# PRONTOLab/GB-25

Measured on AMD Instinct MI355X. Metric: model time-steps/sec, higher is better.
Workload: dtype f32; 1 GPU; baroclinic_instability_model 1440x720x48 LatitudeLongitudeGrid, halo 8, SplitExplicit(30), WENO5, TEOS10, dt=120s; cells_per_gpu=49766400, local_columns=1440, local_rows=720, parallelism=single GPU, rccl_ranks=0

## Files before the change

### gb-25_amd/binding.py

```python
import ctypes as C
import os

import numpy as np

_HERE = os.path.dirname(os.path.abspath(__file__))
LIB_PATH = os.environ.get("GB25_LIB") or os.path.join(_HERE, "libgb25hip.so")
LIB_PATHS = {"Float32": LIB_PATH, "Float64": os.path.join(_HERE, "libgb25hip_f64.so")}
DTYPES = {"Float32": np.float32, "Float64": np.float64}

FIELD_IDS = {
    "u": 0, "v": 1, "w": 2, "T": 3, "S": 4, "pHY": 5,
    "Gn.u": 6, "Gn.v": 7, "Gn.T": 8, "Gn.S": 9,
    "Gm.u": 10, "Gm.v": 11, "Gm.T": 12, "Gm.S": 13,
    "eta": 14, "U": 15, "V": 16,
    "eta_bar": 17, "U_bar": 18, "V_bar": 19,
    "Gn.U": 20, "Gn.V": 21,
    "e": 22, "Gn.e": 23, "Gm.e": 24, "kappa_u": 25, "kappa_c": 26, "kappa_e": 27, "Le": 28, "Jb": 29,
    "previous_u": 30, "previous_v": 31,
}
METRIC2_IDS = ["dxfc", "dxcc", "dxcf", "dxff", "dyfc", "dycc", "dycf", "dyff", "azcc", "azfc", "azcf", "azff", "fff", "phicc"]
METRIC_IDS = {"phif": 0, "phic": 1, "dxc": 2, "dxf": 3, "azc": 4, "azf": 5, "fcor": 6,
              "zf": 7, "zc": 8, "dzc": 9, "dzf": 10, "dy": 11}
ATMOSPHERE_IDS = {"u": 0, "v": 1, "T": 2, "q": 3, "p": 4, "shortwave": 5, "longwave": 6}
KERNEL_IDS = {"fill_halos": 0, "compute_w": 1, "compute_p": 2, "gu": 3, "gv": 4, "tracers": 5,
              "ab2_velocities": 6, "ab2_tracers": 7, "barotropic": 8, "corrector": 9, "implicit": 10, "closure": 11,
              "fluxes": 12, "diagnostics": 13}

ABI_SYMBOLS = [
    "gb25_default_config", "gb25_create", "gb25_destroy", "gb25_last_error_string", "gb25_version",
    "gb25_real_bytes", "gb25_config_bytes", "gb25_catke_parameters_bytes",
    "gb25_set_stream", "gb25_use_own_stream", "gb25_synchronize", "gb25_field_dims", "gb25_set_field", "gb25_get_field",
    "gb25_field_device_ptr", "gb25_get_metric", "gb25_get_metric2", "gb25_get_substepping", "gb25_set_vertical_diffusivity",
    "gb25_get_vertical_diffusivity", "gb25_set_closure_catke", "gb25_set_prescribed_atmosphere",
    "gb25_compute_atmosphere_ocean_fluxes", "gb25_get_top_flux", "gb25_default_catke_parameters",
    "gb25_set_catke_parameters", "gb25_get_catke_parameters", "gb25_set_bottom_drag", "gb25_get_bottom_drag", "gb25_set_tracer_advection_order",
    "gb25_get_tracer_advection_order",
    "gb25_set_baroclinic_instability",
    "gb25_get_clock", "gb25_set_dt", "gb25_initialize", "gb25_mask_immersed_fields",
    "gb25_fill_halo_regions", "gb25_compute_auxiliaries", "gb25_fill_diffusivity_halos",
    "gb25_compute_momentum_tendencies", "gb25_compute_tracer_tendencies", "gb25_compute_boundary_tendencies",
    "gb25_compute_tendencies", "gb25_ab2_step", "gb25_correct_velocities_and_cache_previous_tendencies",
    "gb25_update_state", "gb25_first_time_step", "gb25_time_step", "gb25_loop",
    "gb25_set_option", "gb25_get_option", "gb25_set_bottom_height", "gb25_set_curvilinear_grid", "gb25_set_vertical_faces", "gb25_get_bottom_info", "gb25_set_top_flux",
    "gb25_comm_unique_id", "gb25_comm_init_rccl", "gb25_comm_init_local", "gb25_comm_init_callback", "gb25_comm_finalize",
    "gb25_comm_info", "gb25_debug_exchange_plan",
    "gb25_lookahead_state", "gb25_debug_sequence", "gb25_save_state",
    "gb25_profile_enable", "gb25_profile_reset", "gb25_profile_get",
    "gb25_field_stats_bytes", "gb25_field_diff_bytes", "gb25_state_monitor_bytes", "gb25_get_field_stats", "gb25_compare_field",
    "gb25_get_state_monitor", "gb25_field_device_ptr_readonly",
    "gb25_integrate_field", "gb25_get_budget", "gb25_moments_bytes", "gb25_budget_bytes",
    "gb25_derived_dims", "gb25_compute_derived", "gb25_get_derived", "gb25_get_derived_stats", "gb25_get_field_levels",
    "gb25_transport_bytes", "gb25_get_transport",
    "gb25_class_sum_bytes", "gb25_get_class_sums",
    "gb25_spectral_coefficient_bytes", "gb25_get_spectrum_table", "gb25_get_zonal_spectrum", "gb25_get_derived_zonal_spectrum",
    "gb25_compute_on_surfaces", "gb25_get_on_surfaces",
    "gb25_stability_dims", "gb25_compute_stability", "gb25_get_stability", "gb25_get_stability_stats",
    "gb25_block_info_bytes", "gb25_block_dims", "gb25_derived_block_dims", "gb25_get_block_sums", "gb25_compute_block_sums",
    "gb25_get_derived_block_sums",
    "gb25_averages_info_bytes", "gb25_averages_begin", "gb25_averages_accumulate", "gb25_averages_get_info", "gb25_average_dims",
    "gb25_get_average", "gb25_average_device_ptr", "gb25_averages_end",
    "gb25_particles_info_bytes", "gb25_particles_begin", "gb25_particles_set", "gb25_particles_get", "gb25_particles_advance",
    "gb25_particles_sample", "gb25_particles_get_info", "gb25_particles_end",
]
DERIVED_IDS = {"vorticity": 0, "kinetic_energy": 1, "density_anomaly": 2, "potential_density": 3, "mixed_layer_depth": 4}
SUM_SHAPES = {"rows": 0, "levels": 1, "total": 2}
TRANSPORT_FACES = {"across_y": 0, "across_x": 1}
TRANSPORT_SHAPES = {"lines": 0, "profile": 1, "streamfunction": 2}
CLASS_WHAT = {"faces_y": 0, "cells": 1}
CLASS_VARIABLES = {"T": 0, "S": 1, "potential_density": 2}
# ... 255 lines not shown
    lib.gb25_set_dt.argtypes = [P, C.c_double]
    lib.gb25_ab2_step.argtypes = [P, C.c_double, C.c_int]
    lib.gb25_correct_velocities_and_cache_previous_tendencies.argtypes = [P, C.c_double]
    lib.gb25_loop.argtypes = [P, C.c_int32]
    lib.gb25_save_state.argtypes = [P, C.c_char_p, C.c_char_p]
    lib.gb25_set_top_flux.argtypes = [P, C.c_int, P]
    lib.gb25_set_bottom_height.argtypes = [P, P]
    lib.gb25_set_curvilinear_grid.argtypes = [P, P, C.c_int32, C.c_int32]
    lib.gb25_set_vertical_faces.argtypes = [P, C.POINTER(C.c_double), C.c_int32]
    lib.gb25_get_bottom_info.argtypes = [P, C.c_int32, C.c_int32, C.c_int32, C.POINTER(C.c_double)]
    lib.gb25_set_option.argtypes = [P, C.c_int, C.c_int32]
    lib.gb25_get_option.argtypes = [P, C.c_int, C.POINTER(C.c_int32)]
    lib.gb25_comm_unique_id.argtypes = [P]
    lib.gb25_comm_info.argtypes = [P, C.POINTER(C.c_int32), C.POINTER(C.c_int32)]
    lib.gb25_debug_exchange_plan.argtypes = [C.c_int32, C.c_int32, C.c_int32, C.c_int32, C.c_int32, C.c_char_p, C.c_int64]
    lib.gb25_debug_exchange_plan.restype = C.c_int64
    lib.gb25_comm_init_rccl.argtypes = [P, P]
    lib.gb25_comm_init_local.argtypes = [C.POINTER(P), C.c_int32]
    lib.gb25_comm_init_callback.argtypes = [P, EXCHANGE_FN, P]
    lib.gb25_comm_finalize.argtypes = [P]
    lib.gb25_debug_sequence.argtypes = [C.c_int32, C.c_int32, C.c_int32, C.c_int32, C.c_char_p, C.c_int64]
    lib.gb25_debug_sequence.restype = C.c_int64
    lib.gb25_lookahead_state.argtypes = [P, C.POINTER(C.c_int32), C.POINTER(C.c_int32)]
    lib.gb25_get_field_stats.argtypes = [P, C.c_int, C.c_int, C.POINTER(FieldStats)]
    lib.gb25_compare_field.argtypes = [P, C.c_int, C.c_int, P, C.c_int32, C.POINTER(C.c_int32), C.POINTER(C.c_int32),
                                       C.POINTER(FieldDiff)]
    lib.gb25_get_state_monitor.argtypes = [P, C.POINTER(StateMonitor)]
    lib.gb25_field_device_ptr_readonly.argtypes = [P, C.c_int, C.POINTER(P), C.POINTER(C.c_int32)]
    lib.gb25_integrate_field.argtypes = [P, C.c_int, C.c_int, P, C.c_int64]
    lib.gb25_get_budget.argtypes = [P, C.POINTER(Budget)]
    lib.gb25_derived_dims.argtypes = [P, C.c_int, C.POINTER(C.c_int32)]
    lib.gb25_compute_derived.argtypes = [P, C.c_int, C.c_double, C.c_int32, C.c_int32, C.POINTER(P), C.POINTER(C.c_int32)]
    lib.gb25_get_derived.argtypes = [P, C.c_int, C.c_double, C.c_int32, C.c_int32, P]
    lib.gb25_get_derived_stats.argtypes = [P, C.c_int, C.c_double, C.POINTER(FieldStats)]
    lib.gb25_get_field_levels.argtypes = [P, C.c_int, C.c_int32, C.c_int32, P]
    lib.gb25_get_transport.argtypes = [P, C.c_int, C.c_int, C.c_int32, C.c_int32, P, C.c_int64]
    lib.gb25_get_class_sums.argtypes = [P, C.c_int, C.c_int, P, C.c_int32, C.c_int, C.c_int32, C.c_int32, P, C.c_int64]
    lib.gb25_get_spectrum_table.argtypes = [P, P, P, C.c_int64]
    lib.gb25_get_zonal_spectrum.argtypes = [P, C.c_int, C.c_int32, C.c_int32, C.c_int32, C.c_int32, P, C.c_int64, C.POINTER(C.c_int64)]
    lib.gb25_get_derived_zonal_spectrum.argtypes = [P, C.c_int, C.c_double, C.c_int32, C.c_int32, C.c_int32, C.c_int32, P, C.c_int64,
                                                    C.POINTER(C.c_int64)]
    lib.gb25_compute_on_surfaces.argtypes = [P, C.c_int, C.c_int, P, C.c_int32, C.POINTER(P), C.POINTER(P), C.POINTER(C.c_int32)]
    lib.gb25_get_on_surfaces.argtypes = [P, C.c_int, C.c_int, P, C.c_int32, P, P]
    lib.gb25_stability_dims.argtypes = [P, C.c_int, C.POINTER(C.c_int32)]
    lib.gb25_compute_stability.argtypes = [P, C.c_int, C.c_double, C.c_int32, C.c_int32, C.POINTER(P), C.POINTER(C.c_int32)]
    lib.gb25_get_stability.argtypes = [P, C.c_int, C.c_double, C.c_int32, C.c_int32, P]
# ... 568 lines not shown

    def set_vertical_faces(self, zf):
        a = np.ascontiguousarray(np.asarray(zf, dtype=np.float64))
        self._call("gb25_set_vertical_faces", a.ctypes.data_as(C.POINTER(C.c_double)), int(a.size))

    def bottom_info(self, which, i, j):
        v = C.c_double()
        self._call("gb25_get_bottom_info", {"kbot": 0, "Hfc": 1, "Hcf": 2}[which], i - 1, j - 1, C.byref(v))
        return v.value

    def set_option(self, name, value):
        self._call("gb25_set_option", OPTION_IDS[name], int(value))

    def get_option(self, name):
        v = C.c_int32()
        self._call("gb25_get_option", OPTION_IDS[name], C.byref(v))
        return v.value

    def lookahead_state(self):
        a, b = C.c_int32(), C.c_int32()
        self._call("gb25_lookahead_state", C.byref(a), C.byref(b))
        return bool(a.value), bool(b.value)

    def comm_unique_id(self):
        buf = C.create_string_buffer(UNIQUE_ID_BYTES)
        st = self.lib.gb25_comm_unique_id(buf)
        if st != 0:
            raise GB25Error(f"gb25_comm_unique_id: status {st} (librccl could not be loaded?)")
        return buf.raw

    def comm_init_rccl(self, unique_id):
        if len(unique_id) != UNIQUE_ID_BYTES:
            raise ValueError("unique id must be 128 bytes")
        self._call("gb25_comm_init_rccl", C.c_char_p(bytes(unique_id)))

    def comm_info(self):
        t, n = C.c_int32(0), C.c_int32(0)
        self._call("gb25_comm_info", C.byref(t), C.byref(n))
        return ("none", "rccl", "local", "callback")[t.value], n.value

    def comm_init_callback(self, fn):
        def trampoline(user, b, sw, se, rw, re, nbytes):
            try:
                fn(b, sw, se, rw, re, nbytes)
                return 0
            except Exception as e:
# ... 24 lines not shown
```

### gb-25_amd/csrc/gb25_api.hip

```cpp
#include "../../include/gb25.h"
#include <dlfcn.h>
#include "kernels.hpp"
#include "tendency_kernels.hpp"
#include "diagnostics_kernels.hpp"
#include "averages_kernels.hpp"
#include "class_kernels.hpp"
#include "particle_kernels.hpp"
#include "spectrum_kernels.hpp"
#include "surface_kernels.hpp"
#include "stability_kernels.hpp"
#include "block_kernels.hpp"
#include "diagnostics_state.hpp"
#include "validity.hpp"
#include "step_route.hpp"
#include "subcycle_plan.hpp"

#include <cmath>
#include <cstdarg>
#include <cstdio>
#include <cstdlib>
#include <cstring>
#include <algorithm>
#include <array>
#include <chrono>
#include <condition_variable>
#include <memory>
#include <mutex>
#include <string>
#include <thread>
#include <atomic>
#include <vector>

using namespace gb25;

namespace {

constexpr int PAD = 2;

struct Field {
  real* d = nullptr;
  int nx = 0, ny = 0, nz = 0;
  size_t elems() const { return (size_t)nx * ny * nz; }
};

struct EventPair {
  hipEvent_t a, b;
};

struct DeviceBlocks {
  std::vector<void*> blocks;
  template <class T>
  hipError_t alloc(T** p, size_t bytes, bool zero = false) {
    void* d = nullptr;
    const hipError_t e = hipMalloc(&d, bytes);
    if (e != hipSuccess) return e;
    blocks.push_back(d);
    *p = static_cast<T*>(d);
    return zero ? hipMemset(d, 0, bytes) : hipSuccess;
  }
  template <class T>
  void release(T*& p) {
    blocks.erase(std::remove(blocks.begin(), blocks.end(), static_cast<void*>(p)), blocks.end());
    (void)hipFree(p);
    p = nullptr;
  }
  void release_all() {
    for (void* d : blocks) (void)hipFree(d);
    blocks.clear();
  }
};

}

struct gb25_model {
  gb25_config cfg;
  int Nx = 0;
  int Ny = 0;
  int Rx = 1, Ry = 1, rx = 0, ry = 0, j0 = 0;
  bool ys_open = false, yn_open = false;
  Grid g;
  Field f[GB25_FIELD_COUNT];
  Field pp[3];
  Field dpx, dpy;
  Field colsum[2];
  Field ahead[2];
  Field ahead_uv[2], ahead_G[2], ahead_colsum[2];
  real* uv_partials = nullptr;
  Field pp2[3];
  Field ahead_eta[3], ahead_bar[3];
  real* bars_ahead = nullptr;
  Validity<real> valid;
  bool phy_stale = false;
  int phy_pinned = 0;
  bool baro_inflight = false;
  bool baro_adopted = false;
  int baro_ahead = 1;
  hipEvent_t ev_baro = nullptr, ev_mom = nullptr;
  int fill_fused = 1;
  int ab2_ahead = 1;
  real* bars = nullptr;
  DeviceBlocks mem;
  std::vector<double> h_metric[11];
  std::vector<double> h_curv[GB25_M2_COUNT];
  std::vector<double> host_curv[GB25_M2_COUNT];
  std::vector<double> host_zf, host_bottom;
  int metric_off_j = 0, metric_off_k = 0;
  int Ns = 0;
  double dtau_frac = 0;
  std::vector<double> weights;
  int W = 0, Wy = 0, Wys = 0;
  real* tall_buf = nullptr;
  Field wide[2][3];
  Field wideG[2];
  Field wideBar[3];
  double time = 0, last_dt = 0;
  int64_t iteration = 0;
  hipStream_t own_stream = nullptr, stream = nullptr, side_stream = nullptr;
  hipStream_t baro_stream = nullptr;
  hipEvent_t ev_fork = nullptr, ev_join = nullptr;
  hipEvent_t ev_ts = nullptr, ev_tend = nullptr;
  hipEvent_t ev_strips = nullptr;
  std::array<hipEvent_t*, 7> events() { return {&ev_fork, &ev_join, &ev_baro, &ev_mom, &ev_ts, &ev_tend, &ev_strips}; }
  std::array<hipStream_t*, 3> streams() { return {&own_stream, &side_stream, &baro_stream}; }
  bool strips_issued = false;
  int early_strips = 1;
  int tracers_first = 1;
  int two_streams = 1;
  bool profile = false;
  int profile_only = -1;
  std::vector<EventPair> pending[GB25_K_COUNT];
  std::vector<EventPair> free_events;
  int64_t prof_count[GB25_K_COUNT] = {0};
  int64_t prof_seen[GB25_K_COUNT] = {0};
  double prof_ms[GB25_K_COUNT] = {0};
  std::string err;
  int baro_block = 5;
  int kernel_gen = 2;
  int pressure_form = 0;
  int spectrum_table_where = 0;
  int pressure_bits = 64;
  int n_cu = 256;
  int fold_fills = 1;
  bool composite = false;
  bool ahead_ts_folded = false, ahead_eta_folded = false;
  int split_tendencies = 1;
// ... 792 lines not shown
}

gb25_status compute_w_impl(gb25_model* m, int part = 0) {
  const Grid& g = m->g;
  Timed t(m, GB25_K_COMPUTE_W);
  int ia = -g.H + 1, na = g.Nx + 2 * g.H - 2, ib = 0, nbcols = 0;
  if (part == 1) {
    ia = 0; na = g.Nx - 1;
  } else if (part == 2) {
    ia = -g.H + 1; na = g.H - 1; ib = g.Nx - 1; nbcols = g.H;
  }
  const int ey = g.Ny + 2 * g.H - 2;
  dim3 b = (na + nbcols) >= 64 ? dim3(64, 4) : dim3(16, 16);
  const LazyCorr lz{m->corr[0].d, m->corr[1].d, m->wbase, m->g.sx * m->g.sy_v};
  auto kw = k_compute_w<false, false>;
  if (m->route.kernels_add_correction()) kw = k_compute_w<false, true>;
  else if (g.cv.on) kw = k_compute_w<true, false>;
  hipLaunchKernelGGL(kw, grid2(na + nbcols, ey, b), b, 0, m->stream, g, m->f[GB25_U].d, m->f[GB25_V].d, m->f[GB25_W].d, ia,
                     na, ib, nbcols, lz);
  LAUNCHCHK();
  return GB25_OK;
}
gb25_status compute_p_impl(gb25_model* m, int i_first = INT_MIN, int i_last = INT_MIN, int i_first_b = 0,
                           int i_last_b = -1, bool may_skip_p = false, int j_first = INT_MIN, int j_last = INT_MIN) {
  const Grid& g = m->g;
  const real *Tsrc = m->f[GB25_T].d, *Ssrc = m->f[GB25_S].d;
  real *dpx_out = m->dpx.d, *dpy_out = m->dpy.d;
  if (m->pressure_bits == 32) {
    Timed t(m, GB25_K_COMPUTE_P);
    dim3 b(64, 4);
    const int nx = g.Nx + 2 * g.H - 2, ny = g.Ny + 2 * g.H - 2;
    hipLaunchKernelGGL(k_compute_p_literal, grid2(nx, ny, b), b, 0, m->stream, g, m->f[GB25_T].d, m->f[GB25_S].d,
                       m->f[GB25_PHY].d, -g.H + 1, nx, 0, 0);
    const long n = (long)m->f[GB25_PHY].elems();
    hipLaunchKernelGGL(k_pressure_differences, dim3((unsigned)((n + 255) / 256)), dim3(256), 0, m->stream, g,
                       m->f[GB25_PHY].d, m->dpx.d, m->dpy.d, n);
    m->phy_stale = false;
    LAUNCHCHK();
    return GB25_OK;
  }
  real* n2 = nullptr;
  const bool write_p = !may_skip_p || m->phy_pinned;
  m->phy_stale = !write_p;
  if (i_first == INT_MIN) {
    i_first = -g.H + 1;
    i_last = g.Nx + g.H - 2;
  }
  Timed t(m, GB25_K_COMPUTE_P);
  dim3 b(64, 4);
  const int ncol = i_last - i_first + 2;
  const int ncol_b = i_last_b >= i_first_b ? i_last_b - i_first_b + 2 : 0;
  if (j_first == INT_MIN) {
    j_first = -g.H + 1;
    j_last = g.Ny + g.H - 2;
  }
  const int nrow = j_last - j_first + 1;
  const int tiles_a = (ncol + 62) / 63, tiles_b = (ncol_b + 62) / 63;
  const bool narrow = (tiles_a + tiles_b) * ((nrow + PR * 4 - 1) / (PR * 4)) < 1024;
  const int form = m->pressure_form ? m->pressure_form : (narrow && !g.cv.on && ncol + ncol_b <= 400) ? 1 : narrow ? 2 : 3;
  if (form == 1) {
    const int ta = (i_last - i_first + 1 + 14) / 15, tb = ncol_b ? (i_last_b - i_first_b + 1 + 14) / 15 : 0;
    dim3 gr(ta + tb, (nrow + 11) / 12);
    auto kern = write_p ? k_compute_p_tile<true> : k_compute_p_tile<false>;
    hipLaunchKernelGGL(kern, gr, b, 0, m->stream, g, Tsrc, Ssrc, m->f[GB25_PHY].d, dpx_out, dpy_out, i_first, i_last,
                       i_first_b, i_last_b, ta, n2, j_first, j_last);
  } else if (form == 2) {
    dim3 gr(tiles_a + tiles_b, (nrow + 3) / 4);
    auto kern = write_p ? k_compute_p<1, true> : k_compute_p<1, false>;
    hipLaunchKernelGGL(kern, gr, b, 0, m->stream, g, Tsrc, Ssrc, m->f[GB25_PHY].d, dpx_out, dpy_out, i_first, i_last,
                       i_first_b, i_last_b, tiles_a, n2, j_first, j_last);
  } else {
    dim3 gr(tiles_a + tiles_b, (nrow + PR * 4 - 1) / (PR * 4));
    auto kern = write_p ? k_compute_p<PR, true> : k_compute_p<PR, false>;
    hipLaunchKernelGGL(kern, gr, b, 0, m->stream, g, Tsrc, Ssrc, m->f[GB25_PHY].d, dpx_out, dpy_out, i_first, i_last,
                       i_first_b, i_last_b, tiles_a, n2, j_first, j_last);
  }
  LAUNCHCHK();
  return GB25_OK;
}

void tile_grid(const Grid& g, int* nbx, int* nb) {
  *nbx = (g.Nx + TX - 1) / TX;
  int nby = (g.Ny + TY - 1) / TY;
  *nb = *nbx * nby * g.Nz;
}

inline int interior_tile_columns_end(const Grid& g) {
  const int nbx = (g.Nx + V2_TX - 1) / V2_TX;
  return std::max(1, std::min(nbx - 1, (g.Nx - 3) / V2_TX));
}
inline bool tendencies_split(const gb25_model* m) {
  return m->slab && m->split_tendencies && m->two_streams && m->pressure_bits == 64 && m->kernel_gen >= 2 &&
         interior_tile_columns_end(m->g) > 1 && !m->g.cv.north_fold && m->Ry == 1;
// ... 902 lines not shown
}
inline bool route_carries_w(const gb25_model* m, Corrector c) {
  if (c == Corrector::InConsumers) return m->slab ? slab_wfly_ok(m) : (m->w_fly && chunkings_match(m));
  return c != Corrector::Sweep;
}

struct Cols { int i0, ni, skip_from, skip; };
constexpr Cols NO_COLS{0, 0, INT_MAX, 0};
gb25_status unswept_head(gb25_model* m, dim3 b, Cols c, int jr0, int nj, Cols bases, bool cache) {
  gb25_status s;
  if (c.ni > 0) {
    if ((s = corrector_2d_impl(m, b, c.i0, c.ni, c.skip_from, c.skip, jr0, nj))) return s;
    if (c.skip == 0) m->valid.void_colsums();
  }
  if (!m->route.tracer_kernel_corrects()) m->route.correction_left_in_2d();
  if (bases.ni > 0) {
    if ((s = w_bases_impl(m, b, bases.i0, bases.ni, bases.skip_from, bases.skip))) return s;
    m->route.w_carried_in_kernels();
  }
  if (cache) cache_previous_tendencies(m);
  return GB25_OK;
}

gb25_status time_step_impl(gb25_model* m, int euler, bool more = false) {
  gb25_status s;
  const double dt = m->last_dt;
  struct Composite {
    gb25_model* m;
    explicit Composite(gb25_model* m_) : m(m_) { m->composite = true; }
    ~Composite() { m->composite = false; }
  } composite_scope(m);
  if (!m->two_streams) {
    if ((s = materialize_uv(m))) return s;
    if ((s = ab2_step_impl(m, dt, euler))) return s;
    m->time += dt;
    m->iteration += 1;
    if ((s = fill_halos_impl(m, true))) return s;
    if ((s = corrector_impl(m, true))) return s;
    if ((s = update_state_impl(m))) return s;
    return atmosphere_ocean_fluxes_impl(m);
  }
  const real chi = euler ? -real(0.5) : (real)m->cfg.chi;
  hipStream_t main = m->stream, side = m->side_stream;
  const bool adopted = m->valid.velocities_adoptable((real)dt, chi);
  const bool baro_adopted = adopted && m->valid.ahead_baro_valid;
  m->valid.void_subcycle_lookahead();
  const Corrector corrector = choose_corrector(m, more, adopted, baro_adopted);
  if (corrector != Corrector::InConsumers && (s = materialize_uv(m, corrector == Corrector::Sweep))) return s;
  m->route.begin(corrector, route_carries_w(m, corrector));
  if ((s = ab2_velocities_impl(m, (real)dt, chi))) return s;
  Halo2 hG = halo2_G(m);
  if (!adopted && (s = fill_halos_2d(m, hG))) return s;
  const bool ts_adopted = m->valid.tracers_adoptable((real)dt, chi);
  const bool early_fork = m->valid.take_tend_forkable() && adopted && ts_adopted && !m->catke && m->nu == 0 && m->kappa == 0 &&
                          !m->coupled && !m->g.cv.north_fold;
  HIPCHK(hipEventRecord(m->ev_fork, main));
  HIPCHK(hipStreamWaitEvent(side, early_fork ? m->ev_tend : m->ev_fork, 0));
  const bool complete = m->valid.take_complete_fill();
  {
    OnStream on(m, side);
    if ((s = ab2_tracers_impl(m, (real)dt, chi))) return s;
    if ((complete || !(ts_adopted && m->ahead_ts_folded)) && (s = fill_halos_impl(m, true, false, 1, 2))) return s;
    if (m->catke && m->catke_stale_e_halos && (s = fill_halos_impl(m, true, false, 1, 4))) return s;
    HIPCHK(hipEventRecord(m->ev_ts, side));
    if ((s = compute_p_impl(m, INT_MIN, INT_MIN, 0, -1, true))) return s;
    if (adopted && (s = fill_halos_2d(m, hG))) return s;
  }
  HIPCHK(hipEventRecord(m->ev_join, side));
  bool eta_halos_fresh;
  if (baro_adopted) {
    if (m->baro_inflight) HIPCHK(hipStreamWaitEvent(main, m->ev_baro, 0));
    m->baro_inflight = false;
    adopt_subcycle(m);
    eta_halos_fresh = m->ahead_eta_folded;
  } else {
    const SubcycleDone done = barotropic_impl(m, (real)dt);
    if (done.status) return done.status;
    eta_halos_fresh = done.halo_images_written;
  }
  m->time += dt;
  m->iteration += 1;
  const Grid& g = m->g;
  const dim3 b(64, 4);
  const Cols own{0, g.Nx, INT_MAX, 0}, wide{-2, g.Nx + 4, INT_MAX, 0};
  switch (corrector) {
    case Corrector::InConsumers: {
      Timed t(m, GB25_K_CORRECTOR);
      if ((s = unswept_head(m, b, own, 0, g.Ny + 1, m->route.kernels_carry_w() ? wide : NO_COLS, true))) return s;
// ... 23 lines not shown
      s = corrector_impl(m, true);
      m->route.sweep_done();
      if (s) return s;
      if (corrector == Corrector::SweepWFly && (s = w_bases_impl(m, b, wide.i0, wide.ni, wide.skip_from, wide.skip))) return s;
      if (corrector == Corrector::SweepWFly) m->route.w_carried_in_kernels();
      break;
  }
  {
    const bool unswept = corrector == Corrector::InConsumers || corrector == Corrector::ThroughTracers;
    const bool uv_fresh = unswept || (producers_fold(m) && m->composite && !complete);
    const int which = (uv_fresh ? 0 : 1) | ((eta_halos_fresh && !complete) ? 0 : 2);
    if (which && (s = fill_halos_impl(m, true, false, which, 1))) return s;
  }
  if (!m->route.kernels_carry_w() && (s = compute_w_impl(m))) return s;
  if (corrector == Corrector::ThroughTracers && !m->tracers_first) return fail(m, GB25_ERR_STATE, "internal: the corrector through the tracer kernel needs the tracer kernel first");
  const bool tracers_first = m->tracers_first != 0;
  if (m->catke) {
    HIPCHK(hipStreamWaitEvent(main, m->ev_ts, 0));
    if ((s = catke_update_impl(m))) return s;
  }
  if (tracers_first) {
    HIPCHK(hipStreamWaitEvent(main, m->ev_ts, 0));
    if ((s = tracers_impl(m))) return s;
  }
  HIPCHK(hipStreamWaitEvent(main, m->ev_join, 0));
  if ((s = momentum_impl(m))) return s;
  if (tracers_first) {
    HIPCHK(hipEventRecord(m->ev_tend, main));
    m->valid.tendencies_forkable();
  }
  if (m->valid.velocities_ready(m->baro_ahead)) {
    if (m->baro_ahead == 2) {
      if (!m->baro_stream) HIPCHK(hipStreamCreateWithFlags(&m->baro_stream, hipStreamNonBlocking));
      HIPCHK(hipEventRecord(m->ev_mom, main));
      HIPCHK(hipStreamWaitEvent(m->baro_stream, m->ev_mom, 0));
      {
        OnStream on(m, m->baro_stream);
        const SubcycleDone done = barotropic_impl(m, m->valid.ahead_uv_dt, true);
        s = done.status;
        m->ahead_eta_folded = done.halo_images_written;
      }
      if (s) return s;
      HIPCHK(hipEventRecord(m->ev_baro, m->baro_stream));
      m->baro_inflight = true;
    } else {
      const SubcycleDone done = barotropic_impl(m, m->valid.ahead_uv_dt, true);
// ... 97 lines not shown
  m->cfg = *cfg;
  m->Ry = cfg->ranks_y > 1 ? cfg->ranks_y : 1;
  if (cfg->Nx < 8 || cfg->Ny < 8 || cfg->Nz < 4 || cfg->halo < 4 || cfg->substeps < 1 || cfg->substeps > 4096 ||
      cfg->nranks < 1 || cfg->rank < 0 || cfg->rank >= cfg->nranks || cfg->nranks % m->Ry != 0 ||
      cfg->Nx % (cfg->nranks / m->Ry) != 0 || cfg->Ny % m->Ry != 0)
    return fail(m, GB25_ERR_INVALID_ARGUMENT,
                "invalid configuration: need Nx,Ny >= 8, Nz >= 4, halo >= 4, 1 <= substeps <= 4096, nranks = Rx ranks_y, "
                "Nx %% Rx == 0, Ny %% ranks_y == 0");
  if (cfg->slab_mode < 0 || cfg->slab_mode > 1)
    return fail(m, GB25_ERR_INVALID_ARGUMENT, "slab_mode must be 0 (x halos by exchange iff nranks > 1) or 1 (always)");
  m->Rx = cfg->nranks / m->Ry;
  m->rx = cfg->rank % m->Rx;
  m->ry = cfg->rank / m->Rx;
  m->Nx = cfg->Nx / m->Rx;
  m->Ny = cfg->Ny / m->Ry;
  m->j0 = m->ry * m->Ny;
  m->ys_open = m->ry > 0;
  m->yn_open = m->ry < m->Ry - 1;
  m->slab = cfg->nranks > 1 || cfg->slab_mode == 1;
  {
    const int nbx = (m->Nx + 63) / 64, nby = (m->Ny + 3) / 4;
    if ((long)nbx * nby * std::max(1, cfg->Nz / 24) >= 4096) m->mom_chunk_levels = m->trc_chunk_levels = 24;
  }
  if (const char* rows = getenv("GB25_TRACER_ROWS")) {
    if (strcmp(rows, "1") != 0 && strcmp(rows, "2") != 0)
      return fail(m, GB25_ERR_INVALID_ARGUMENT, "GB25_TRACER_ROWS must be 1 or 2 (unset: the library's rule)");
    m->tracer_rows_forced = rows[0] - '0';
  }
  if (m->Nx < cfg->halo) return fail(m, GB25_ERR_INVALID_ARGUMENT, "slab narrower than the halo");
  if (m->Ry > 1) {
    m->split_tendencies = 0;
    if (m->Ny < cfg->halo + 2) return fail(m, GB25_ERR_INVALID_ARGUMENT, "a rank's band of rows is narrower than the halo");
  }
  {
    const double plane = (double)(m->Nx + 2 * cfg->halo) * (m->Ny + 2 * cfg->halo + 1);
    const double elems = plane * (cfg->Nz + 2 * cfg->halo + 1);
    const int kchunks = std::max(1, cfg->Nz / 12), klen = (cfg->Nz + kchunks - 1) / kchunks;
    if (elems >= 2147483648.0 || plane * (klen + 10) * sizeof(real) >= 2147483648.0)
      return fail(m, GB25_ERR_INVALID_ARGUMENT,
                  "a %dx%dx%d slab has %.2g elements per 3-D array (%.1f GB) and %.2g per plane; the kernels index at most 2^31 "
                  "elements per array and %d planes of 2 GB together: decompose in x (nranks) so that the local slab is narrower",
                  m->Nx, m->Ny, cfg->Nz, elems, elems * sizeof(real) / 1e9, plane, klen + 10);
  }
  int ndev = 0;
  if (hipGetDeviceCount(&ndev) != hipSuccess || ndev == 0)
    return fail(m, GB25_ERR_NO_DEVICE, "no HIP device visible; libgb25hip has no CPU fallback");
// ... 259 lines not shown
  return s;
}
gb25_status gb25_get_field(gb25_model* m, gb25_field f, void* host_, int include_halos) {
  real* host = static_cast<real*>(host_);
  if (m && f == GB25_PHY && m->phy_stale) {
    gb25_status s = compute_p_impl(m);
    if (s) return s;
  }
  return copy_field(m, f, host, include_halos, false);
}
gb25_status gb25_field_device_ptr(gb25_model* m, gb25_field id, void** dev) {
  if (!m || id < 0 || id >= GB25_FIELD_COUNT || !dev) return GB25_ERR_INVALID_ARGUMENT;
  if (!m->f[id].d) return fail(m, GB25_ERR_INVALID_ARGUMENT, "this model has no such field (closure = CATKEVerticalDiffusivity() only)");
  if (gb25_status s = collective_guard(m, 2, (unsigned)id, 0.0)) return s;
  if (m->route.memory_lacks_correction())
    if (gb25_status s = materialize_uv(m)) return s;
  if (gb25_status s = materialize_prev_uv(m)) return s;
  if (id == GB25_U || id == GB25_V || id == GB25_T || id == GB25_S || (id >= GB25_GN_U && id <= GB25_GM_S) ||
      (id >= GB25_ETA && id <= GB25_GN_BT_V)) {
    m->valid.pointer_handed_out();
  }
  if (id == GB25_PHY) {
    m->phy_pinned = true;
    if (m->phy_stale) {
      gb25_status s = compute_p_impl(m);
      if (s) return s;
    }
  }
  *dev = m->f[id].d;
  return GB25_OK;
}
gb25_status gb25_get_metric(const gb25_model* m, gb25_metric id, int32_t logical_index, double* v) {
  if (!m || id < 0 || id > GB25_M_DY || !v) return GB25_ERR_INVALID_ARGUMENT;
  if (id == GB25_M_DY) {
    *v = (double)m->g.dy;
    return GB25_OK;
  }
  int off = (id <= GB25_M_FCOR) ? m->metric_off_j : m->metric_off_k;
  long a = (long)logical_index - 1 + off;
  if (a < 0 || a >= (long)m->h_metric[id].size()) return GB25_ERR_INVALID_ARGUMENT;
  *v = (double)(real)m->h_metric[id][a];
  return GB25_OK;
}
gb25_status gb25_get_metric2(const gb25_model* m, gb25_metric2 id, double* v, int64_t count) {
  if (!m || id < 0 || id >= GB25_M2_COUNT || !v) return GB25_ERR_INVALID_ARGUMENT;
  const std::vector<double>& a = m->h_curv[id];
// ... 586 lines not shown
}
static gb25_status loop_impl(gb25_model* m, int32_t n);
gb25_status gb25_time_step(gb25_model* m) {
  CHECK_MODEL(m);
  Range r_step(m, "time_step");
  return loop_impl(m, 1);
}
gb25_status gb25_loop(gb25_model* m, int32_t n) {
  CHECK_MODEL(m);
  Range r_loop(m, "loop");
  return loop_impl(m, n);
}
static gb25_status loop_impl(gb25_model* m, int32_t n) {
  if (m->slab) {
    if (gb25_status s = need_group(m, "gb25_loop")) return s;
    GroupOps ops(*m->group);
    for (int it = 0; it < n; it++)
      if (gb25_status s = sequence_time_step(ops, 0, m->group->lookahead_in_flight)) return s;
    for (gb25_model* q : m->group->slabs)
      if (gb25_status s = materialize_uv(q)) return fail(m, s, "%s", q->err.c_str());
    return GB25_OK;
  }
  for (int it = 0; it < n; it++)
    if (gb25_status s = time_step_impl(m, 0, true)) return s;
  return materialize_uv(m);
}

gb25_status gb25_lookahead_state(const gb25_model* m, int32_t* velocities_ready, int32_t* subcycle_adopted) {
  if (!m) return GB25_ERR_INVALID_ARGUMENT;
  if (velocities_ready) *velocities_ready = m->valid.velocities_ready(m->baro_ahead) ? 1 : 0;
  if (subcycle_adopted) *subcycle_adopted = m->baro_adopted ? 1 : 0;
  return GB25_OK;
}

int64_t gb25_debug_sequence(int32_t nslabs, int32_t first, int32_t adopted, int32_t ready, char* out, int64_t cap) {
  if (nslabs < 1) return -1;
  TraceOps ops(nslabs, adopted != 0, ready != 0);
  if (first & 2) ops.fold = true;
  if (first & 4) ops.is_coupled = true;
  if (first & 64) ops.early = true;
  if (first & 32) ops.is_lazy = true;
  if (first & 16) ops.mesh = true;
  if (first & 128) ops.is_catke = true;
  bool in_flight = (first & 8) != 0;
  first &= 1;
  if (first) sequence_first_time_step(ops, in_flight);
  else sequence_time_step(ops, 0, in_flight);
  ops.add("lookahead_in_flight %d", in_flight ? 1 : 0);
  const int64_t need = (int64_t)ops.log.size() + 1;
  if (out && cap > 0) {
// ... 82 lines not shown
```

### gb-25_amd/csrc/kernels.hpp

```cpp
#pragma once
#include "device_common.hpp"
#include "subcycle_plan.hpp"

namespace gb25 {

__device__ __forceinline__ void store_x_images(const Grid& g, real* a, int o, real x, bool xw, bool xe) {
  a[o] = x;
  if (xw) a[o + g.Nx] = x;
  if (xe) a[o - g.Nx] = x;
}

constexpr int TX = 64, TY = 4;

struct TileIdx {
  int i, j, k;
  bool ok;
};
__device__ __forceinline__ TileIdx tile_index(const Grid& g, int nbx, int nb) {
  int L = xcd_remap(blockIdx.x, nb);
  int bx = L % nbx, r = L / nbx;
  int k = r % g.Nz, by = r / g.Nz;
  TileIdx t;
  t.i = bx * TX + threadIdx.x;
  t.j = by * TY + threadIdx.y;
// ... 287 lines not shown
  w[o] = real(0.);
  real due = real(0.), duw = real(0.), dvn = real(0.), dvs = real(0.);
  if (LAZY) {
    due = lz.du[o2 + 1]; duw = lz.du[o2];
    dvn = lz.dv[o2 + g.sx]; dvs = lz.dv[o2];
  }
#pragma unroll 8
  for (int k = 0; k < g.Nz; k++) {
    real dz = uniform_at(g.dzc, k);
    real div = LAZY ? (dye * dz * (u[o + 1] + due) - dyw * dz * (u[o] + duw)) + (dxn * dz * (v[ov + g.sx] + dvn) - dxs * dz * (v[ov] + dvs))
                    : (dye * dz * u[o + 1] - dyw * dz * u[o]) + (dxn * dz * v[ov + g.sx] - dxs * dz * v[ov]);
    wk = wk - div * raz;
    o += g.pl_c;
    ov += g.pl_v;
    w[o] = wk;
  }
}

constexpr int PR = 4;
#ifndef GB25_P_MINW
#define GB25_P_MINW 1
#endif
template <int PR_, bool WRITE_P>
__global__ __launch_bounds__(256, GB25_P_MINW) void k_compute_p(Grid g, const real* __restrict__ T, const real* __restrict__ S,
                                                   real* __restrict__ p, real* __restrict__ dpx,
                                                   real* __restrict__ dpy, int i_first, int i_last, int i_first_b,
                                                   int i_last_b, int tiles_a, real* __restrict__ n2, int j_first, int j_last) {
  const int lane = threadIdx.x;
  const bool second = (int)blockIdx.x >= tiles_a;
  if (second) {
    i_first = i_first_b;
    i_last = i_last_b;
  }
  const int i = i_first - 1 + ((int)blockIdx.x - (second ? tiles_a : 0)) * 63 + lane;
  const int jb = j_first + (blockIdx.y * blockDim.y + threadIdx.y) * PR_;
  const int imax = i_last, jmax = j_last;
  if (jb > jmax) return;
  const int ic_ = min(i, g.Nx + g.H - 1);
  const int Nz = g.Nz;
  const double gr = -(double)g.g / (double)g.rho0;
  const double sc = 0.875 / 35.16504;
  int o[PR_ + 1];
  double bup[PR_ + 1], pk[PR_ + 1];
#pragma unroll
  for (int r = 0; r <= PR_; r++) {
    const int j = min(jb - 1 + r, g.Ny + g.H - 1);
    o[r] = ic(g, ic_, j, Nz);
    bup[r] = gr * teos10_level(g.eos + 28 * Nz, sqrt_pos(((double)S[o[r]] + 32.0) * sc), (double)T[o[r]] * 0.025);
    pk[r] = 0.0;
  }
  for (int k = Nz - 1; k >= 0; k--) {
    const double* c = g.eos + 28 * k;
    const double dz = g.dzf_d[k + 1];
#pragma unroll
    for (int r = 0; r <= PR_; r++) {
      o[r] -= g.pl_c;
      double bk = gr * teos10_level(c, sqrt_pos(((double)S[o[r]] + 32.0) * sc), (double)T[o[r]] * 0.025);
      pk[r] = pk[r] - 0.5 * (bk + bup[r]) * dz;
      bup[r] = bk;
    }
#pragma unroll
    for (int r = 1; r <= PR_; r++) {
      const double pw = __shfl_up(pk[r], 1);
      const int j = jb - 1 + r;
      if (lane >= 1 && i <= imax && j <= jmax) {
        if (WRITE_P) p[o[r]] = (real)pk[r];
        dpx[o[r]] = (real)(pk[r] - pw);
        dpy[o[r]] = (real)(pk[r] - pk[r - 1]);
      }
    }
  }
}
template <bool WRITE_P>
__global__ __launch_bounds__(256) void k_compute_p_tile(Grid g, const real* __restrict__ T, const real* __restrict__ S,
                                                        real* __restrict__ p, real* __restrict__ dpx, real* __restrict__ dpy,
                                                        int i_first, int i_last, int i_first_b, int i_last_b, int tiles_a,
                                                        real* __restrict__ n2, int j_first, int j_last) {
  const int lane = threadIdx.x, lx = lane & 15, ly = lane >> 4;
  const bool second = (int)blockIdx.x >= tiles_a;
  if (second) {
    i_first = i_first_b;
    i_last = i_last_b;
  }
  const int i = i_first - 1 + ((int)blockIdx.x - (second ? tiles_a : 0)) * 15 + lx;
  const int j = j_first - 1 + (int)(blockIdx.y * blockDim.y + threadIdx.y) * 3 + ly;
  if (j_first + (int)(blockIdx.y * blockDim.y + threadIdx.y) * 3 > j_last) return;
  const int Nz = g.Nz;
  const double gr = -(double)g.g / (double)g.rho0;
  const double sc = 0.875 / 35.16504;
  int o = ic(g, min(i, g.Nx + g.H - 1), min(j, g.Ny + g.H - 1), Nz);
  const bool writes = lx >= 1 && ly >= 1 && i <= i_last && j <= j_last;
  double bup = gr * teos10_level(g.eos + 28 * Nz, sqrt_pos(((double)S[o] + 32.0) * sc), (double)T[o] * 0.025);
  double pk = 0.0;
  for (int k = Nz - 1; k >= 0; k--) {
// ... 1458 lines not shown
```

### gb-25_amd/csrc/validity.hpp

```cpp
#pragma once
namespace {
template <class Real> struct Validity {
  bool ahead_valid = false, ahead_uv_valid = false, ahead_baro_valid = false;
  Real ahead_dt = 0, ahead_chi = 0, ahead_uv_dt = 0, ahead_uv_chi = 0;
  bool colsum_valid = false;
  bool halo_colsum_valid = false;
  bool tend_forkable = false;
  int complete_fills_needed = 2;
  bool ptr_exposed = false;
  void void_lookaheads() { ahead_valid = ahead_uv_valid = ahead_baro_valid = false; }
  void void_tracer_lookahead() { ahead_valid = false; }
  void void_velocity_lookaheads() { ahead_uv_valid = ahead_baro_valid = false; }
  void void_velocity_lookahead_alone() { ahead_uv_valid = false; }
  void void_subcycle_lookahead() { ahead_baro_valid = false; }
  void void_colsums() { colsum_valid = false; }
  void complete_fills_owed() { complete_fills_needed = 2; }
  void option_changes() { void_lookaheads(); tend_forkable = false; }
  void pointer_handed_out() { ptr_exposed = true; void_lookaheads(); }
  void grid_changes() { option_changes(); colsum_valid = halo_colsum_valid = false; complete_fills_owed(); }
  void tendency_kernel_runs(bool from_new_state) { tend_forkable = false; if (from_new_state) void_velocity_lookaheads(); }
  void record_tracer_lookahead(bool made, Real dt, Real chi) { ahead_valid = made; ahead_dt = dt; ahead_chi = chi; }
  void record_velocity_lookahead(Real dt, Real chi) { ahead_uv_valid = true; ahead_uv_dt = dt; ahead_uv_chi = chi; }
  void record_subcycle_lookahead() { ahead_baro_valid = true; }
  void record_colsums() { colsum_valid = true; }
  void halo_colsums_packed() { halo_colsum_valid = colsum_valid; }
  void tendencies_forkable() { tend_forkable = true; }
  bool take_tend_forkable() { const bool was = tend_forkable; tend_forkable = false; return was; }
  bool take_complete_fill() { return complete_fills_needed > 0 ? (complete_fills_needed -= 1, true) : false; }
  bool tracers_adoptable(Real dt, Real chi) const { return ahead_valid && dt == ahead_dt && chi == ahead_chi; }
  bool velocities_adoptable(Real dt, Real chi) const { return ahead_uv_valid && dt == ahead_uv_dt && chi == ahead_uv_chi; }
  bool velocities_ready(int subcycle_lookahead) const { return ahead_uv_valid && subcycle_lookahead && !ptr_exposed; }
};
}
```

### include/gb25.h

```cpp
#ifndef GB25_H
#define GB25_H

#include <stddef.h>
#include <stdint.h>

#ifdef __cplusplus
extern "C" {
#endif

typedef struct gb25_model gb25_model;

typedef enum {
  GB25_OK = 0,
  GB25_ERR_INVALID_ARGUMENT = 1,
  GB25_ERR_HIP = 2,
  GB25_ERR_OUT_OF_MEMORY = 3,
  GB25_ERR_NO_DEVICE = 4,
  GB25_ERR_STATE = 5,
  GB25_ERR_COMM = 6
} gb25_status;

typedef enum {
  GB25_U = 0, GB25_V, GB25_W, GB25_T, GB25_S, GB25_PHY,
  GB25_GN_U, GB25_GN_V, GB25_GN_T, GB25_GN_S,
// ... 162 lines not shown
gb25_status gb25_compute_momentum_tendencies(gb25_model *m);
gb25_status gb25_compute_tracer_tendencies(gb25_model *m);
gb25_status gb25_compute_boundary_tendencies(gb25_model *m);
gb25_status gb25_compute_tendencies(gb25_model *m);
gb25_status gb25_ab2_step(gb25_model *m, double dt, int euler);
gb25_status gb25_correct_velocities_and_cache_previous_tendencies(gb25_model *m, double dt);
gb25_status gb25_update_state(gb25_model *m);

gb25_status gb25_first_time_step(gb25_model *m);
gb25_status gb25_time_step(gb25_model *m);
gb25_status gb25_loop(gb25_model *m, int32_t n_inner);

#define GB25_UNIQUE_ID_BYTES 128
gb25_status gb25_comm_unique_id(void *id_out);
gb25_status gb25_comm_init_rccl(gb25_model *m, const void *unique_id);
gb25_status gb25_comm_init_local(gb25_model *const *slabs, int32_t n);
typedef int32_t (*gb25_exchange_fn)(void *user, int32_t buffer_set, const void *send_west, const void *send_east,
                                    void *recv_west, void *recv_east, int64_t nbytes);
gb25_status gb25_comm_init_callback(gb25_model *m, gb25_exchange_fn fn, void *user);
gb25_status gb25_comm_finalize(gb25_model *m);
gb25_status gb25_comm_info(const gb25_model *m, int32_t *transport, int32_t *comm_ranks);
int64_t gb25_debug_exchange_plan(int32_t Rx, int32_t Ry, int32_t rank, int32_t folded_grid, int32_t group, char *out, int64_t cap);
gb25_status gb25_lookahead_state(const gb25_model *m, int32_t *velocities_ready, int32_t *subcycle_adopted);
int64_t gb25_debug_sequence(int32_t nslabs, int32_t first, int32_t adopted, int32_t ready, char *out, int64_t cap);

gb25_status gb25_save_state(gb25_model *m, const char *directory, const char *label);

typedef struct {
  double min, max, max_abs, sum, sum_sq;
  int64_t count, nonfinite;
  int32_t at_max_abs[3], first_nonfinite[3], global_offset[3];
  int32_t reserved;
} gb25_field_stats;
typedef struct {
  double max_abs_a, max_abs_b, max_abs_delta, sum_sq_a, sum_sq_b, sum_sq_delta;
  int64_t count, nonfinite;
  int32_t at_max_abs_delta[3], global_offset[3];
} gb25_field_diff;
typedef struct {
  gb25_field_stats u, v, w, eta, T, S;
  double cfl;
  int32_t at_cfl[3], reserved;
  int64_t nonfinite_total, iteration;
  double time;
} gb25_state_monitor;
int32_t gb25_field_stats_bytes(void);
// ... 169 lines not shown
```

Baseline: 456.5 steps/s.

## Compute next step's pressure gradients early on side stream from lookahead tracers

```diff
diff --git a/gb-25_amd/binding.py b/gb-25_amd/binding.py
--- a/gb-25_amd/binding.py
+++ b/gb-25_amd/binding.py
@@ -44,7 +44,7 @@
     "gb25_set_option", "gb25_get_option", "gb25_set_bottom_height", "gb25_set_curvilinear_grid", "gb25_set_vertical_faces", "gb25_get_bottom_info", "gb25_set_top_flux",
     "gb25_comm_unique_id", "gb25_comm_init_rccl", "gb25_comm_init_local", "gb25_comm_init_callback", "gb25_comm_finalize",
     "gb25_comm_info", "gb25_debug_exchange_plan",
-    "gb25_lookahead_state", "gb25_debug_sequence", "gb25_save_state",
+    "gb25_lookahead_state", "gb25_early_pressure_state", "gb25_debug_sequence", "gb25_save_state",
     "gb25_profile_enable", "gb25_profile_reset", "gb25_profile_get",
     "gb25_field_stats_bytes", "gb25_field_diff_bytes", "gb25_state_monitor_bytes", "gb25_get_field_stats", "gb25_compare_field",
     "gb25_get_state_monitor", "gb25_field_device_ptr_readonly",
@@ -346,6 +346,7 @@
     lib.gb25_debug_sequence.argtypes = [C.c_int32, C.c_int32, C.c_int32, C.c_int32, C.c_char_p, C.c_int64]
     lib.gb25_debug_sequence.restype = C.c_int64
     lib.gb25_lookahead_state.argtypes = [P, C.POINTER(C.c_int32), C.POINTER(C.c_int32)]
+    lib.gb25_early_pressure_state.argtypes = [P, C.POINTER(C.c_int32), C.POINTER(C.c_int32), C.POINTER(C.c_int64)]
     lib.gb25_get_field_stats.argtypes = [P, C.c_int, C.c_int, C.POINTER(FieldStats)]
     lib.gb25_compare_field.argtypes = [P, C.c_int, C.c_int, P, C.c_int32, C.POINTER(C.c_int32), C.POINTER(C.c_int32),
                                        C.POINTER(FieldDiff)]
@@ -960,6 +961,11 @@
         self._call("gb25_lookahead_state", C.byref(a), C.byref(b))
         return bool(a.value), bool(b.value)
 
+    def early_pressure_state(self):
+        a, b, n = C.c_int32(), C.c_int32(), C.c_int64()
+        self._call("gb25_early_pressure_state", C.byref(a), C.byref(b), C.byref(n))
+        return bool(a.value), b.value, n.value
+
     def comm_unique_id(self):
         buf = C.create_string_buffer(UNIQUE_ID_BYTES)
         st = self.lib.gb25_comm_unique_id(buf)
diff --git a/gb-25_amd/csrc/gb25_api.hip b/gb-25_amd/csrc/gb25_api.hip
--- a/gb-25_amd/csrc/gb25_api.hip
+++ b/gb-25_amd/csrc/gb25_api.hip
@@ -36,6 +36,12 @@
 namespace {
 
 constexpr int PAD = 2;
+#ifndef GB25_EARLY_PRESSURE_DEFAULT
+#define GB25_EARLY_PRESSURE_DEFAULT 1
+#endif
+#ifndef GB25_EARLY_P_BLOCKS_DEFAULT
+#define GB25_EARLY_P_BLOCKS_DEFAULT 256
+#endif
 
 struct Field {
   real* d = nullptr;
@@ -82,6 +88,9 @@
   Field f[GB25_FIELD_COUNT];
   Field pp[3];
   Field dpx, dpy;
+  Field dp_next[2];
+  int early_pressure = GB25_EARLY_PRESSURE_DEFAULT, early_p_blocks = GB25_EARLY_P_BLOCKS_DEFAULT;
+  int64_t early_p_adopted = 0;
   Field colsum[2];
   Field ahead[2];
   Field ahead_uv[2], ahead_G[2], ahead_colsum[2];
@@ -119,8 +128,9 @@
   hipStream_t baro_stream = nullptr;
   hipEvent_t ev_fork = nullptr, ev_join = nullptr;
   hipEvent_t ev_ts = nullptr, ev_tend = nullptr;
+  hipEvent_t ev_trc = nullptr;
   hipEvent_t ev_strips = nullptr;
-  std::array<hipEvent_t*, 7> events() { return {&ev_fork, &ev_join, &ev_baro, &ev_mom, &ev_ts, &ev_tend, &ev_strips}; }
+  std::array<hipEvent_t*, 8> events() { return {&ev_fork, &ev_join, &ev_baro, &ev_mom, &ev_ts, &ev_tend, &ev_strips, &ev_trc}; }
   std::array<hipStream_t*, 3> streams() { return {&own_stream, &side_stream, &baro_stream}; }
   bool strips_issued = false;
   int early_strips = 1;
@@ -959,10 +969,12 @@
   return GB25_OK;
 }
 gb25_status compute_p_impl(gb25_model* m, int i_first = INT_MIN, int i_last = INT_MIN, int i_first_b = 0,
-                           int i_last_b = -1, bool may_skip_p = false, int j_first = INT_MIN, int j_last = INT_MIN) {
+                           int i_last_b = -1, bool may_skip_p = false, int j_first = INT_MIN, int j_last = INT_MIN, bool early = false) {
   const Grid& g = m->g;
-  const real *Tsrc = m->f[GB25_T].d, *Ssrc = m->f[GB25_S].d;
-  real *dpx_out = m->dpx.d, *dpy_out = m->dpy.d;
+  const real *Tsrc = early ? m->ahead[0].d : m->f[GB25_T].d, *Ssrc = early ? m->ahead[1].d : m->f[GB25_S].d;
+  real *dpx_out = early ? m->dp_next[0].d : m->dpx.d, *dpy_out = early ? m->dp_next[1].d : m->dpy.d;
+  if (early && (m->pressure_bits != 64 || !may_skip_p || m->phy_pinned || !dpx_out || !dpy_out))
+    return fail(m, GB25_ERR_STATE, "internal: an early pressure launch that would store pHY' or has no arrays");
   if (m->pressure_bits == 32) {
     Timed t(m, GB25_K_COMPUTE_P);
     dim3 b(64, 4);
@@ -978,7 +990,7 @@
   }
   real* n2 = nullptr;
   const bool write_p = !may_skip_p || m->phy_pinned;
-  m->phy_stale = !write_p;
+  if (!early) m->phy_stale = !write_p;
   if (i_first == INT_MIN) {
     i_first = -g.H + 1;
     i_last = g.Nx + g.H - 2;
@@ -1006,6 +1018,10 @@
     auto kern = write_p ? k_compute_p<1, true> : k_compute_p<1, false>;
     hipLaunchKernelGGL(kern, gr, b, 0, m->stream, g, Tsrc, Ssrc, m->f[GB25_PHY].d, dpx_out, dpy_out, i_first, i_last,
                        i_first_b, i_last_b, tiles_a, n2, j_first, j_last);
+  } else if (early && m->early_p_blocks > 0) {
+    const int tiles_x = tiles_a + tiles_b, ntiles = tiles_x * ((nrow + PR * 4 - 1) / (PR * 4));
+    hipLaunchKernelGGL((k_compute_p_walk<PR, false>), dim3(m->early_p_blocks), b, 0, m->stream, g, Tsrc, Ssrc, m->f[GB25_PHY].d, dpx_out,
+                       dpy_out, i_first, i_last, i_first_b, i_last_b, tiles_a, j_first, j_last, tiles_x, ntiles);
   } else {
     dim3 gr(tiles_a + tiles_b, (nrow + PR * 4 - 1) / (PR * 4));
     auto kern = write_p ? k_compute_p<PR, true> : k_compute_p<PR, false>;
@@ -1954,7 +1970,7 @@
   return GB25_OK;
 }
 
-gb25_status time_step_impl(gb25_model* m, int euler, bool more = false) {
+gb25_status time_step_impl(gb25_model* m, int euler, bool more = false, bool another_follows = false) {
   gb25_status s;
   const double dt = m->last_dt;
   struct Composite {
@@ -1989,13 +2005,19 @@
   HIPCHK(hipEventRecord(m->ev_fork, main));
   HIPCHK(hipStreamWaitEvent(side, early_fork ? m->ev_tend : m->ev_fork, 0));
   const bool complete = m->valid.take_complete_fill();
+  const bool p_early = m->valid.take_early_pressure((real)dt, chi);
   {
     OnStream on(m, side);
     if ((s = ab2_tracers_impl(m, (real)dt, chi))) return s;
     if ((complete || !(ts_adopted && m->ahead_ts_folded)) && (s = fill_halos_impl(m, true, false, 1, 2))) return s;
     if (m->catke && m->catke_stale_e_halos && (s = fill_halos_impl(m, true, false, 1, 4))) return s;
     HIPCHK(hipEventRecord(m->ev_ts, side));
-    if ((s = compute_p_impl(m, INT_MIN, INT_MIN, 0, -1, true))) return s;
+    if (p_early) {
+      std::swap(m->dpx.d, m->dp_next[0].d);
+      std::swap(m->dpy.d, m->dp_next[1].d);
+      m->phy_stale = true;
+      m->early_p_adopted += 1;
+    } else if ((s = compute_p_impl(m, INT_MIN, INT_MIN, 0, -1, true))) return s;
     if (adopted && (s = fill_halos_2d(m, hG))) return s;
   }
   HIPCHK(hipEventRecord(m->ev_join, side));
@@ -2065,6 +2087,19 @@
   if (tracers_first) {
     HIPCHK(hipStreamWaitEvent(main, m->ev_ts, 0));
     if ((s = tracers_impl(m))) return s;
+    if (m->early_pressure && another_follows && early_fork && !complete && m->valid.complete_fills_needed == 0 && m->ahead_ts_folded &&
+        m->valid.tracers_adoptable((real)m->last_dt, (real)m->cfg.chi) && corrector == Corrector::InConsumers && !m->slab &&
+        !m->immersed && !g.cv.on && m->pressure_bits == 64 && !m->phy_pinned) {
+      for (int q = 0; q < 2; q++)
+        if (!m->dp_next[q].d && (s = alloc_field(m, m->dp_next[q], m->dpx.nx, m->dpx.ny, m->dpx.nz))) return s;
+      HIPCHK(hipEventRecord(m->ev_trc, main));
+      HIPCHK(hipStreamWaitEvent(side, m->ev_trc, 0));
+      {
+        OnStream on(m, side);
+        if ((s = compute_p_impl(m, INT_MIN, INT_MIN, 0, -1, true, INT_MIN, INT_MIN, true))) return s;
+      }
+      m->valid.record_early_pressure();
+    }
   }
   HIPCHK(hipStreamWaitEvent(main, m->ev_join, 0));
   if ((s = momentum_impl(m))) return s;
@@ -2208,6 +2243,18 @@
     const int nbx = (m->Nx + 63) / 64, nby = (m->Ny + 3) / 4;
     if ((long)nbx * nby * std::max(1, cfg->Nz / 24) >= 4096) m->mom_chunk_levels = m->trc_chunk_levels = 24;
   }
+  if (const char* on = getenv("GB25_EARLY_PRESSURE")) {
+    if (strcmp(on, "0") != 0 && strcmp(on, "1") != 0)
+      return fail(m, GB25_ERR_INVALID_ARGUMENT, "GB25_EARLY_PRESSURE must be 0 or 1 (unset: the library's default)");
+    m->early_pressure = on[0] - '0';
+  }
+  if (const char* blocks = getenv("GB25_EARLY_P_BLOCKS")) {
+    char* end = nullptr;
+    const long G = strtol(blocks, &end, 10);
+    if (end == blocks || *end || G < 0 || G > 65535)
+      return fail(m, GB25_ERR_INVALID_ARGUMENT, "GB25_EARLY_P_BLOCKS must be a block count in 0 .. 65535 (0: the plain launch; unset: the library's default)");
+    m->early_p_blocks = (int)G;
+  }
   if (const char* rows = getenv("GB25_TRACER_ROWS")) {
     if (strcmp(rows, "1") != 0 && strcmp(rows, "2") != 0)
       return fail(m, GB25_ERR_INVALID_ARGUMENT, "GB25_TRACER_ROWS must be 1 or 2 (unset: the library's rule)");
@@ -2513,6 +2560,7 @@
   }
   if (id == GB25_PHY) {
     m->phy_pinned = true;
+    m->valid.pressure_pinned();
     if (m->phy_stale) {
       gb25_status s = compute_p_impl(m);
       if (s) return s;
@@ -3145,10 +3193,17 @@
     return GB25_OK;
   }
   for (int it = 0; it < n; it++)
-    if (gb25_status s = time_step_impl(m, 0, true)) return s;
+    if (gb25_status s = time_step_impl(m, 0, true, it + 1 < n)) return s;
   return materialize_uv(m);
 }
 
+gb25_status gb25_early_pressure_state(const gb25_model* m, int32_t* enabled, int32_t* blocks, int64_t* adopted_steps) {
+  if (!m) return GB25_ERR_INVALID_ARGUMENT;
+  if (enabled) *enabled = m->early_pressure;
+  if (blocks) *blocks = m->early_p_blocks;
+  if (adopted_steps) *adopted_steps = m->early_p_adopted;
+  return GB25_OK;
+}
 gb25_status gb25_lookahead_state(const gb25_model* m, int32_t* velocities_ready, int32_t* subcycle_adopted) {
   if (!m) return GB25_ERR_INVALID_ARGUMENT;
   if (velocities_ready) *velocities_ready = m->valid.velocities_ready(m->baro_ahead) ? 1 : 0;
diff --git a/gb-25_amd/csrc/kernels.hpp b/gb-25_amd/csrc/kernels.hpp
--- a/gb-25_amd/csrc/kernels.hpp
+++ b/gb-25_amd/csrc/kernels.hpp
@@ -333,18 +333,18 @@
 #define GB25_P_MINW 1
 #endif
 template <int PR_, bool WRITE_P>
-__global__ __launch_bounds__(256, GB25_P_MINW) void k_compute_p(Grid g, const real* __restrict__ T, const real* __restrict__ S,
-                                                   real* __restrict__ p, real* __restrict__ dpx,
-                                                   real* __restrict__ dpy, int i_first, int i_last, int i_first_b,
-                                                   int i_last_b, int tiles_a, real* __restrict__ n2, int j_first, int j_last) {
+__device__ __forceinline__ void compute_p_block(const Grid& g, const real* __restrict__ T, const real* __restrict__ S,
+                                                real* __restrict__ p, real* __restrict__ dpx, real* __restrict__ dpy, int i_first,
+                                                int i_last, int i_first_b, int i_last_b, int tiles_a, int j_first, int j_last,
+                                                const int bx, const int by) {
   const int lane = threadIdx.x;
-  const bool second = (int)blockIdx.x >= tiles_a;
+  const bool second = bx >= tiles_a;
   if (second) {
     i_first = i_first_b;
     i_last = i_last_b;
   }
-  const int i = i_first - 1 + ((int)blockIdx.x - (second ? tiles_a : 0)) * 63 + lane;
-  const int jb = j_first + (blockIdx.y * blockDim.y + threadIdx.y) * PR_;
+  const int i = i_first - 1 + (bx - (second ? tiles_a : 0)) * 63 + lane;
+  const int jb = j_first + (by * blockDim.y + threadIdx.y) * PR_;
   const int imax = i_last, jmax = j_last;
   if (jb > jmax) return;
   const int ic_ = min(i, g.Nx + g.H - 1);
@@ -381,6 +381,23 @@
       }
     }
   }
+}
+template <int PR_, bool WRITE_P>
+__global__ __launch_bounds__(256, GB25_P_MINW) void k_compute_p(Grid g, const real* __restrict__ T, const real* __restrict__ S,
+                                                   real* __restrict__ p, real* __restrict__ dpx,
+                                                   real* __restrict__ dpy, int i_first, int i_last, int i_first_b,
+                                                   int i_last_b, int tiles_a, real* __restrict__ n2, int j_first, int j_last) {
+  compute_p_block<PR_, WRITE_P>(g, T, S, p, dpx, dpy, i_first, i_last, i_first_b, i_last_b, tiles_a, j_first, j_last, (int)blockIdx.x,
+                                (int)blockIdx.y);
+}
+template <int PR_, bool WRITE_P>
+__global__ __launch_bounds__(256, GB25_P_MINW) void k_compute_p_walk(Grid g, const real* __restrict__ T, const real* __restrict__ S,
+                                                   real* __restrict__ p, real* __restrict__ dpx, real* __restrict__ dpy,
+                                                   int i_first, int i_last, int i_first_b, int i_last_b, int tiles_a,
+                                                   int j_first, int j_last, int tiles_x, int ntiles) {
+  for (int tile = blockIdx.x; tile < ntiles; tile += gridDim.x)
+    compute_p_block<PR_, WRITE_P>(g, T, S, p, dpx, dpy, i_first, i_last, i_first_b, i_last_b, tiles_a, j_first, j_last,
+                                  tile % tiles_x, tile / tiles_x);
 }
 template <bool WRITE_P>
 __global__ __launch_bounds__(256) void k_compute_p_tile(Grid g, const real* __restrict__ T, const real* __restrict__ S,
diff --git a/gb-25_amd/csrc/validity.hpp b/gb-25_amd/csrc/validity.hpp
--- a/gb-25_amd/csrc/validity.hpp
+++ b/gb-25_amd/csrc/validity.hpp
@@ -8,26 +8,30 @@
   bool tend_forkable = false;
   int complete_fills_needed = 2;
   bool ptr_exposed = false;
-  void void_lookaheads() { ahead_valid = ahead_uv_valid = ahead_baro_valid = false; }
-  void void_tracer_lookahead() { ahead_valid = false; }
+  bool early_p_valid = false;
+  void void_lookaheads() { ahead_valid = ahead_uv_valid = ahead_baro_valid = early_p_valid = false; }
+  void void_tracer_lookahead() { ahead_valid = early_p_valid = false; }
+  void pressure_pinned() { early_p_valid = false; }
   void void_velocity_lookaheads() { ahead_uv_valid = ahead_baro_valid = false; }
   void void_velocity_lookahead_alone() { ahead_uv_valid = false; }
   void void_subcycle_lookahead() { ahead_baro_valid = false; }
   void void_colsums() { colsum_valid = false; }
-  void complete_fills_owed() { complete_fills_needed = 2; }
+  void complete_fills_owed() { complete_fills_needed = 2; early_p_valid = false; }
   void option_changes() { void_lookaheads(); tend_forkable = false; }
   void pointer_handed_out() { ptr_exposed = true; void_lookaheads(); }
   void grid_changes() { option_changes(); colsum_valid = halo_colsum_valid = false; complete_fills_owed(); }
   void tendency_kernel_runs(bool from_new_state) { tend_forkable = false; if (from_new_state) void_velocity_lookaheads(); }
-  void record_tracer_lookahead(bool made, Real dt, Real chi) { ahead_valid = made; ahead_dt = dt; ahead_chi = chi; }
+  void record_tracer_lookahead(bool made, Real dt, Real chi) { ahead_valid = made; ahead_dt = dt; ahead_chi = chi; early_p_valid = false; }
   void record_velocity_lookahead(Real dt, Real chi) { ahead_uv_valid = true; ahead_uv_dt = dt; ahead_uv_chi = chi; }
   void record_subcycle_lookahead() { ahead_baro_valid = true; }
+  void record_early_pressure() { early_p_valid = ahead_valid; }
   void record_colsums() { colsum_valid = true; }
   void halo_colsums_packed() { halo_colsum_valid = colsum_valid; }
   void tendencies_forkable() { tend_forkable = true; }
   bool take_tend_forkable() { const bool was = tend_forkable; tend_forkable = false; return was; }
   bool take_complete_fill() { return complete_fills_needed > 0 ? (complete_fills_needed -= 1, true) : false; }
   bool tracers_adoptable(Real dt, Real chi) const { return ahead_valid && dt == ahead_dt && chi == ahead_chi; }
+  bool take_early_pressure(Real dt, Real chi) { const bool was = early_p_valid && tracers_adoptable(dt, chi); early_p_valid = false; return was; }
   bool velocities_adoptable(Real dt, Real chi) const { return ahead_uv_valid && dt == ahead_uv_dt && chi == ahead_uv_chi; }
   bool velocities_ready(int subcycle_lookahead) const { return ahead_uv_valid && subcycle_lookahead && !ptr_exposed; }
 };
diff --git a/include/gb25.h b/include/gb25.h
--- a/include/gb25.h
+++ b/include/gb25.h
@@ -208,6 +208,7 @@
 gb25_status gb25_comm_info(const gb25_model *m, int32_t *transport, int32_t *comm_ranks);
 int64_t gb25_debug_exchange_plan(int32_t Rx, int32_t Ry, int32_t rank, int32_t folded_grid, int32_t group, char *out, int64_t cap);
 gb25_status gb25_lookahead_state(const gb25_model *m, int32_t *velocities_ready, int32_t *subcycle_adopted);
+gb25_status gb25_early_pressure_state(const gb25_model *m, int32_t *enabled, int32_t *blocks, int64_t *adopted_steps);
 int64_t gb25_debug_sequence(int32_t nslabs, int32_t first, int32_t adopted, int32_t ready, char *out, int64_t cap);
 
 gb25_status gb25_save_state(gb25_model *m, const char *directory, const char *label);
```

After: 445.6 steps/s. 0.976x the previous value.
